# CatchMan1/AI-education-generative-recommendation

Hardware: AMD Instinct MI355X
Metric: RQ-VAE items encoded/s + SASRec seqs scored/s @1/8 GPU; HR@10/NDCG@10 parity (higher is better)
Workload: dtype f32; 1 GPU; rq_c2: RQ-VAE get_indices, 3x256 codebooks, in 768 -> [256,128] -> e 32, data-derived codebooks, BERT-statistics item embeddings; global_batch=100000, parallelism=item-sharded x1, no collective

## Files before the change

### ai-education-generative-recommendation_amd/csrc/rq_fused.hip

```cpp
#include <type_traits>

#include "gr_common.h"

#ifndef GR_EDIAG
#define GR_EDIAG 0
#endif

namespace gr {

constexpr int FT = 32;
constexpr int FP = 2;
constexpr int FXC = 64;
constexpr int FXP = FXC + 4;
constexpr int FWV = 8;

template <int H1, int H2>
struct FusedCfg {
  static constexpr int E = 32;
  static constexpr int NTH = 64 * FWV;
  static constexpr int P1 = H1 + 4, P2 = H2 + 4, P3 = H2 + 4;
  static constexpr int PI = FP * FT;
  static constexpr int XV = PI * 16 / NTH;
  static constexpr int LDS = 2 * PI * FXP + PI * P1 + PI * P2 + E * P3;
  static_assert(H1 == 32 * FWV && H2 == 128, "8-wave form: H1 = 256, H2 = 128");
};

__device__ __forceinline__ f32x4 ldg4(const float* p) {
  return *reinterpret_cast<const __attribute__((address_space(1))) f32x4*>(reinterpret_cast<uintptr_t>(p));
}

__device__ __forceinline__ void put_packed(float* row, int k0, const f32x4& v) {
  const int g = k0 & ~31, q = k0 & 31, j = q >> 3, e2 = (q >> 1) & 2;
  *reinterpret_cast<f32x2*>(row + g + 4 * j + e2) = f32x2{v[0], v[2]};
  *reinterpret_cast<f32x2*>(row + g + 16 + 4 * j + e2) = f32x2{v[1], v[3]};
}

__device__ __forceinline__ int xrow(int f) { return ((f >> 7) << 3) + ((f >> 5) & 3) + 4 * ((f >> 4) & 1); }

template <int H1, int H2>
struct FusedCtx {
  using C = FusedCfg<H1, H2>;
  const float* x;
  int64_t n;
  int D0, NC, csplit, t_end;
  const float *W2, *b1, *b2, *W3, *b3;
  float* z_out;
  float *xs, *h1s, *h2s, *w3s;
  int tid, w, r, h;
  const float* w1row;
  f32x4 awc[4];
  f32x4 awc2[4];
  f32x4 w2f[4];
  f32x4 xr[C::XV];
  bool xok[C::XV];
  f32x4 bxa[4];
  int buf;
  __device__ __forceinline__ void gload_x(int tb, int c, bool ks) {
#pragma unroll
    for (int i = 0; i < C::XV; ++i) {
      const int f = tid + C::NTH * i, it = xrow(f), k4 = (f & 15) * 4;
      const int64_t item = (int64_t)tb * FT + (ks ? it % FT : it);
      xok[i] = item < n && (ks || (tb + it / FT) < t_end);
      xr[i] = *reinterpret_cast<const f32x4*>(x + (item < n ? item : n - 1) * D0 +
                                              (int64_t)c * FXC + k4 + (ks && it >= FT ? csplit * FXC : 0));
    }
  }
  __device__ __forceinline__ void read_bxa(int g) {
    const float* xb = xs + buf * C::PI * FXP + r * FXP + 16 * h + g * 32;
#pragma unroll
    for (int j = 0; j < 4; ++j) bxa[j] = *reinterpret_cast<const f32x4*>(xb + 4 * j);
  }
  __device__ __forceinline__ void swrite_x(int b) {
#pragma unroll
    for (int i = 0; i < C::XV; ++i) {
      const int f = tid + C::NTH * i;
      put_packed(xs + b * C::PI * FXP + xrow(f) * FXP, (f & 15) * 4,
                 xok[i] ? xr[i] : f32x4{0.f, 0.f, 0.f, 0.f});
    }
  }
};

__device__ __forceinline__ int h1_swz(int row) { return ((row >> 2) ^ (row >> 3)) & 1; }

__device__ __forceinline__ void store_h1(float* row, int x, int g4, int h, const f32x4& o) {
  float* p = row + 16 * (g4 >> 1) + 2 * (g4 & 1) + h;
#pragma unroll
  for (int i = 0; i < 4; ++i) p[4 * (i ^ x)] = o[i];
}

template <int NR, int H1, int H2>
__device__ __forceinline__ void rq_l23(FusedCtx<H1, H2>& cx, int tb) {
#pragma clang fp contract(off)
  using C = FusedCfg<H1, H2>;
  constexpr int E = C::E, P1 = C::P1, P2 = C::P2;
  const int w = cx.w, lane = cx.tid & 63, j = lane & 15, g = lane >> 4;
  f32x4 bb3;
  {
    constexpr int NT = 2 * NR, UB = 4, NI = H1 / (16 * UB);
    f32x4 acc2[NT];
#pragma unroll
    for (int it = 0; it < NT; ++it) acc2[it] = f32x4{0.f, 0.f, 0.f, 0.f};
    const float* hb = cx.h1s + j * P1 + 4 * (g ^ h1_swz(j));
    const float* w2row = cx.W2 + (int64_t)(w * 16 + j) * H1 + 4 * g;
    f32x4 aw2[UB];
#pragma unroll
    for (int u = 0; u < UB; ++u) aw2[u] = cx.w2f[u];
    const f32x4 bb = ldg4(cx.b2 + w * 16 + 4 * g);
    bb3 = ldg4(cx.b3 + 16 * (w & 1) + 4 * g);
    asm volatile("" ::: "memory");
#pragma unroll 1
    for (int bi = 0; bi < (GR_EDIAG == 1 ? 0 : NI); ++bi) {
      const int bn = (bi + 1 < NI) ? bi + 1 : bi;
      f32x4 awn[UB];
#pragma unroll
      for (int u = 0; u < UB; ++u) awn[u] = ldg4(w2row + 16 * (bn * UB + u));
      f32x4 bx[UB][NT];
#pragma unroll
      for (int u = 0; u < UB; ++u)
#pragma unroll
        for (int it = 0; it < NT; ++it)
          bx[u][it] = *reinterpret_cast<const f32x4*>(hb + it * 16 * P1 + 16 * (bi * UB + u));
#pragma unroll
      for (int u = 0; u < UB; ++u)
#pragma unroll
        for (int t = 0; t < 4; ++t)
#pragma unroll
          for (int it = 0; it < NT; ++it) acc2[it] = mfma16(aw2[u][t], bx[u][it][t], acc2[it]);
      __builtin_amdgcn_sched_group_barrier(0x100, NT, 0);
#pragma unroll
      for (int i = 0; i < UB; ++i) {
        __builtin_amdgcn_sched_group_barrier(0x008, 1, 0);
        __builtin_amdgcn_sched_group_barrier(0x020, 1, 0);
      }
#pragma unroll
      for (int i = 0; i < (UB - 1) * NT; ++i) {
        __builtin_amdgcn_sched_group_barrier(0x008, 1, 0);
        __builtin_amdgcn_sched_group_barrier(0x100, 1, 0);
      }
      __builtin_amdgcn_sched_group_barrier(0x008, 4 * UB * NT - UB - (UB - 1) * NT, 0);
#pragma unroll
      for (int u = 0; u < UB; ++u) aw2[u] = awn[u];
    }
#pragma unroll
    for (int it = 0; it < NT; ++it) {
      float* row = cx.h2s + (it * 16 + j) * P2 + w * 16 + g;
#pragma unroll
      for (int i = 0; i < 4; ++i) {
        const float u = bb[i] + acc2[it][i];
        row[4 * i] = u < 0.f ? 0.f : u;
      }
    }
  }
  __syncthreads();

  if (GR_EDIAG != 2 && w < 4 * NR) {
    const int it = w >> 2, ih = (w >> 1) & 1, oh = w & 1;
    f32x4 acc3 = {0.f, 0.f, 0.f, 0.f};
    const float* hb = cx.h2s + (it * FT + 16 * ih + j) * P2 + 4 * g;
    const float* w3row = cx.w3s + (16 * oh + j) * C::P3 + 4 * g;
#pragma unroll
    for (int b = 0; b < H2 / 16; ++b) {
      const f32x4 aw = *reinterpret_cast<const f32x4*>(w3row + 16 * b);
      const f32x4 bx = *reinterpret_cast<const f32x4*>(hb + 16 * b);
#pragma unroll
      for (int t = 0; t < 4; ++t) acc3 = mfma16(aw[t], bx[t], acc3);
    }
    const int64_t item = (int64_t)(tb + it) * FT + 16 * ih + j;
    if (item < cx.n) {
      f32x4 o;
#pragma unroll
      for (int i = 0; i < 4; ++i) o[i] = bb3[i] + acc3[i];
      *reinterpret_cast<f32x4*>(cx.z_out + item * E + 16 * oh + 4 * g) = o;
    }
  }
}

template <int NP, int H1, int H2, bool KS = false>
__device__ __forceinline__ void rq_fused_pass(FusedCtx<H1, H2>& cx, int tb, int next_tb, bool next_ks) {
#pragma clang fp contract(off)
  using C = FusedCfg<H1, H2>;
  constexpr int P1 = C::P1, PI = C::PI;
  static_assert(!KS || NP == 2, "k-split pass: two chains");
  constexpr int NR = KS ? 1 : NP;
  const int w = cx.w, r = cx.r, h = cx.h;
  const int NC = KS ? cx.NC / 2 : cx.NC;
  const int kbo = cx.csplit * FXC;
  asm volatile("" : "+s"(cx.W2), "+s"(cx.W3), "+s"(cx.b1), "+s"(cx.b2), "+s"(cx.b3));

  f32x16 acc1[NP];
#pragma unroll
  for (int it = 0; it < NP; ++it)
#pragma unroll
    for (int v = 0; v < 16; ++v) acc1[it][v] = 0.f;
  constexpr int M1 = 16 * NP;
  const float* xsrc[C::XV];
  const float* xnxt[C::XV];
  bool xok_cur[C::XV], xok_nxt[C::XV];
#pragma unroll
  for (int i = 0; i < C::XV; ++i) {
    const int f = cx.tid + C::NTH * i, it = xrow(f), k4 = (f & 15) * 4;
    const int64_t a = (int64_t)tb * FT + (KS ? it % FT : it);
    const int64_t b = next_tb < 0 ? cx.n : (int64_t)next_tb * FT + (next_ks ? it % FT : it);
    xsrc[i] = cx.x + (a < cx.n ? a : cx.n - 1) * cx.D0 + k4 + (KS && it >= FT ? kbo : 0);
    xnxt[i] = cx.x + (b < cx.n ? b : cx.n - 1) * cx.D0 + k4 + (next_ks && it >= FT ? kbo : 0);
    xok_cur[i] = a < cx.n;
    xok_nxt[i] = b < cx.n && (next_ks || (next_tb + it / FT) < cx.t_end);
    if (b >= cx.n) xnxt[i] = cx.x + (cx.n - 1) * cx.D0 + k4;
  }
  auto group = [&](auto gsel, int c) {
    constexpr int g = decltype(gsel)::value;
    const int gi = 2 * c + g;
    const int gn = (gi + 1 == 2 * NC) ? 0 : gi + 1;
    f32x4 awn[4], awn2[4];
#pragma unroll
    for (int j = 0; j < 4; ++j) awn[j] = *reinterpret_cast<const f32x4*>(cx.w1row + gn * 32 + 4 * j);
    if constexpr (KS) {
#pragma unroll
      for (int j = 0; j < 4; ++j) awn2[j] = *reinterpret_cast<const f32x4*>(cx.w1row + kbo + gn * 32 + 4 * j);
    }
    const float* xb = cx.xs + cx.buf * PI * FXP + r * FXP + 16 * h + g * 32;
    f32x4 bx[NP][4];
#pragma unroll
    for (int j = 0; j < 4; ++j) bx[0][j] = cx.bxa[j];
#pragma unroll
    for (int it = 1; it < NP; ++it)
#pragma unroll
      for (int j = 0; j < 4; ++j) bx[it][j] = *reinterpret_cast<const f32x4*>(xb + it * FT * FXP + 4 * j);
    if constexpr (g == 0) {
      cx.read_bxa(1);
      asm volatile("" ::: "memory");
      const bool same = c + 1 < NC;
#pragma unroll
      for (int i = 0; i < C::XV; ++i)
        cx.xr[i] = *reinterpret_cast<const f32x4*>(same ? xsrc[i] + (c + 1) * FXC : xnxt[i]);
    }
#pragma unroll
    for (int it = 0; it < NP; ++it)
#pragma unroll
      for (int j = 0; j < 4; ++j)
#pragma unroll
        for (int s = 0; s < 4; ++s)
          acc1[it] = mfma32(KS && it == 1 ? cx.awc2[j][s] : cx.awc[j][s], bx[it][j][s], acc1[it]);
    if constexpr (g == 1) {
      const bool same = c + 1 < NC;
#pragma unroll
      for (int i = 0; i < C::XV; ++i) {
        const int f = cx.tid + C::NTH * i;
        const bool ok = same ? xok_cur[i] : xok_nxt[i];
        put_packed(cx.xs + (cx.buf ^ 1) * PI * FXP + xrow(f) * FXP, (f & 15) * 4,
                   ok ? cx.xr[i] : f32x4{0.f, 0.f, 0.f, 0.f});
      }
    }
    constexpr int NX = (g == 0) ? C::XV : 0, NDW = (g == 1) ? 2 * C::XV : 0;
    constexpr int NW = KS ? 8 : 4, NA = (g == 0) ? 4 : 0;
    static_assert(NW + 4 * (NP - 1) + NA + NX + 2 * NDW <= M1, "schedule");
    {
#pragma unroll
      for (int i = 0; i < NW; ++i) {
        __builtin_amdgcn_sched_group_barrier(0x008, 1, 0);
        __builtin_amdgcn_sched_group_barrier(0x020, 1, 0);
      }
#pragma unroll
      for (int i = 0; i < 4 * (NP - 1) + NA; ++i) {
        __builtin_amdgcn_sched_group_barrier(0x008, 1, 0);
        __builtin_amdgcn_sched_group_barrier(0x100, 1, 0);
      }
#pragma unroll
      for (int i = 0; i < NX; ++i) {
        __builtin_amdgcn_sched_group_barrier(0x008, 1, 0);
        __builtin_amdgcn_sched_group_barrier(0x020, 1, 0);
      }
      __builtin_amdgcn_sched_group_barrier(0x008, M1 - NW - 4 * (NP - 1) - NA - NX - 2 * NDW, 0);
#pragma unroll
      for (int i = 0; i < NDW; ++i) {
        __builtin_amdgcn_sched_group_barrier(0x008, 1, 0);
        __builtin_amdgcn_sched_group_barrier(0x200, 1, 0);
      }
    }
#pragma unroll
    for (int j = 0; j < 4; ++j) cx.awc[j] = awn[j];
    if constexpr (KS) {
#pragma unroll
      for (int j = 0; j < 4; ++j) cx.awc2[j] = awn2[j];
    }
  };
  const int f0 = w * 32;
  auto chunk = [&](int c) {
    group(std::integral_constant<int, 0>{}, c);
    group(std::integral_constant<int, 1>{}, c);
    __syncthreads();
    cx.buf ^= 1;
    cx.read_bxa(0);
    __builtin_amdgcn_sched_group_barrier(0x100, 4, 0);
    __builtin_amdgcn_sched_group_barrier(0x008, 2 * C::XV, 0);
  };
  int c = 0;
  f32x16 part[NP];
  f32x4 b1f[4];
#pragma unroll
  for (int g4 = 0; g4 < 4; ++g4) b1f[g4] = ldg4(cx.b1 + f0 + 8 * g4 + 4 * h);
  asm volatile("" ::: "memory");
  if constexpr (KS) {
#pragma unroll
    for (int j = 0; j < 4; ++j) cx.awc2[j] = *reinterpret_cast<const f32x4*>(cx.w1row + kbo + 4 * j);
#pragma unroll 1
    for (; c < NC; ++c) chunk(c);
#pragma unroll
    for (int g4 = 0; g4 < 4; ++g4) {
      const f32x4 bb = b1f[g4];
#pragma unroll
      for (int i = 0; i < 4; ++i) part[0][4 * g4 + i] = bb[i] + acc1[0][4 * g4 + i];
    }
#pragma unroll
    for (int v = 0; v < 16; ++v) acc1[0][v] = acc1[1][v];
  } else {
#pragma unroll 1
    for (; c < cx.csplit; ++c) chunk(c);
#pragma unroll
    for (int g4 = 0; g4 < 4; ++g4) {
      const f32x4 bb = b1f[g4];
#pragma unroll
      for (int it = 0; it < NP; ++it)
#pragma unroll
        for (int i = 0; i < 4; ++i) part[it][4 * g4 + i] = bb[i] + acc1[it][4 * g4 + i];
    }
#pragma unroll
    for (int it = 0; it < NP; ++it)
#pragma unroll
      for (int v = 0; v < 16; ++v) acc1[it][v] = 0.f;
#pragma unroll 1
    for (; c < NC; ++c) chunk(c);
  }
#pragma unroll
  for (int g4 = 0; g4 < 4; ++g4)
#pragma unroll
    for (int it = 0; it < NR; ++it) {
      f32x4 o;
#pragma unroll
      for (int i = 0; i < 4; ++i) {
        const float u = part[it][4 * g4 + i] + acc1[it][4 * g4 + i];
        o[i] = u < 0.f ? 0.f : u;
      }
      store_h1(cx.h1s + (it * FT + r) * P1 + f0, h1_swz(r), g4, h, o);
    }
  __syncthreads();

  rq_l23<NR, H1, H2>(cx, tb);
}

template <int H1, int H2, int PF = 128>
__device__ __forceinline__ void rq_piece_pass(FusedCtx<H1, H2>& cx, int tb, int fh, float* __restrict__ h1g,
                                              const float* __restrict__ W1) {
#pragma clang fp contract(off)
  using C = FusedCfg<H1, H2>;
  constexpr int PI = C::PI;
  constexpr int NG = PF / 32;
  const int w = cx.w, r = cx.r, h = cx.h, fg = w % NG, blk = (w / NG) & 1;
  const bool act = w < 2 * NG;
  const int NC = cx.NC / 2, kbo = cx.csplit * FXC;
  const int f0 = PF * fh + 32 * fg;
  const float* w1row = W1 + (int64_t)(f0 + r) * cx.D0 + 16 * h + blk * kbo;
  f32x4 awc[4];
#pragma unroll
  for (int j = 0; j < 4; ++j) awc[j] = act ? *reinterpret_cast<const f32x4*>(w1row + 4 * j) : f32x4{0.f, 0.f, 0.f, 0.f};
  const float* xsrc[C::XV];
  bool xok[C::XV];
#pragma unroll
  for (int i = 0; i < C::XV; ++i) {
    const int f = cx.tid + C::NTH * i, it = xrow(f), k4 = (f & 15) * 4;
    const int64_t a = (int64_t)tb * FT + it % FT;
    xsrc[i] = cx.x + (a < cx.n ? a : cx.n - 1) * cx.D0 + k4 + (it >= FT ? kbo : 0);
    xok[i] = a < cx.n;
  }
  f32x16 acc;
#pragma unroll
  for (int v = 0; v < 16; ++v) acc[v] = 0.f;
#pragma unroll 1
  for (int c = 0; c < NC; ++c) {
    const bool more = c + 1 < NC;
#pragma unroll
    for (int g = 0; g < 2; ++g) {
      const int gi = 2 * c + g;
      const int gn = gi + 1 < 2 * NC ? gi + 1 : gi;
      f32x4 awn[4];
#pragma unroll
      for (int j = 0; j < 4; ++j)
        awn[j] = act ? *reinterpret_cast<const f32x4*>(w1row + gn * 32 + 4 * j) : f32x4{0.f, 0.f, 0.f, 0.f};
      const float* xb = cx.xs + cx.buf * PI * FXP + (blk * FT + r) * FXP + 16 * h + g * 32;
      f32x4 bx[4];
#pragma unroll
      for (int j = 0; j < 4; ++j) bx[j] = *reinterpret_cast<const f32x4*>(xb + 4 * j);
      if (g == 0 && more) {
#pragma unroll
        for (int i = 0; i < C::XV; ++i) cx.xr[i] = *reinterpret_cast<const f32x4*>(xsrc[i] + (c + 1) * FXC);
      }
      if (act) {
#pragma unroll
        for (int j = 0; j < 4; ++j)
#pragma unroll
          for (int s = 0; s < 4; ++s) acc = mfma32(awc[j][s], bx[j][s], acc);
      }
      if (g == 1 && more) {
#pragma unroll
        for (int i = 0; i < C::XV; ++i) {
          const int f = cx.tid + C::NTH * i;
          put_packed(cx.xs + (cx.buf ^ 1) * PI * FXP + xrow(f) * FXP, (f & 15) * 4,
                     xok[i] ? cx.xr[i] : f32x4{0.f, 0.f, 0.f, 0.f});
        }
      }
#pragma unroll
      for (int j = 0; j < 4; ++j) awc[j] = awn[j];
    }
    __syncthreads();
    cx.buf ^= 1;
  }
  float* hand = cx.h1s + (fg * 64 + (cx.tid & 63)) * 16;
  if (act && blk == 1) {
#pragma unroll
    for (int v4 = 0; v4 < 4; ++v4)
      *reinterpret_cast<f32x4*>(hand + 4 * v4) = f32x4{acc[4 * v4], acc[4 * v4 + 1], acc[4 * v4 + 2], acc[4 * v4 + 3]};
  }
  __syncthreads();
  if (act && blk == 0) {
    const int64_t item = (int64_t)tb * FT + r;
#pragma unroll
    for (int g4 = 0; g4 < 4; ++g4) {
      const f32x4 bb = ldg4(cx.b1 + f0 + 8 * g4 + 4 * h);
      const f32x4 a1 = *reinterpret_cast<const f32x4*>(hand + 4 * g4);
      f32x4 o;
#pragma unroll
      for (int i = 0; i < 4; ++i) {
        const float part = bb[i] + acc[4 * g4 + i];
        const float u = part + a1[i];
        o[i] = u < 0.f ? 0.f : u;
      }
      if (item < cx.n) *reinterpret_cast<f32x4*>(h1g + (int64_t)r * H1 + f0 + 8 * g4 + 4 * h) = o;
    }
  }
  __syncthreads();
}

template <int H1, int H2>
__global__ __launch_bounds__(64 * FWV, 1) void rq_encoder_kernel(
    const float* __restrict__ x, int64_t n, int D0, int csplit, const float* __restrict__ W1,
    const float* __restrict__ b1, const float* __restrict__ W2, const float* __restrict__ b2,
    const float* __restrict__ W3, const float* __restrict__ b3, float* __restrict__ z_out,
    int tiles, float* __restrict__ h1g, int pq) {
  using C = FusedCfg<H1, H2>;
  extern __shared__ __attribute__((aligned(16))) float sm[];
  const int G = gridDim.x, q = tiles / G, b = blockIdx.x;
  const int npieces = (h1g && GR_EDIAG != 3) ? pq * (tiles - q * G) : 0;
  const int t_begin = h1g ? b * q : (int)((int64_t)b * tiles / G);
  const int t_end = h1g ? t_begin + q : (int)((int64_t)(b + 1) * tiles / G);
  const int piece0 = b < npieces ? b : -1;
  const bool pieces_only = t_begin >= t_end;
  if (pieces_only && piece0 < 0) return;
  FusedCtx<H1, H2> cx;
  cx.x = x; cx.n = n; cx.D0 = D0; cx.NC = D0 / FXC; cx.csplit = csplit; cx.t_end = t_end;
  cx.W2 = W2; cx.b1 = b1; cx.b2 = b2; cx.W3 = W3; cx.b3 = b3; cx.z_out = z_out;
  cx.xs = sm;
  cx.h1s = sm + 2 * C::PI * FXP;
  cx.h2s = cx.h1s + C::PI * C::P1;
  cx.w3s = cx.h2s + C::PI * C::P2;
  for (int f = threadIdx.x; f < C::E * H2 / 4; f += C::NTH) {
    const int row = f / (H2 / 4), qq = f % (H2 / 4);
    *reinterpret_cast<f32x4*>(cx.w3s + row * C::P3 + 4 * qq) = *reinterpret_cast<const f32x4*>(W3 + row * H2 + 4 * qq);
  }
  const int tid = threadIdx.x, lane = tid & 63;
  cx.tid = tid; cx.w = tid >> 6; cx.r = lane & 31; cx.h = lane >> 5;
  cx.w1row = W1 + (int64_t)(cx.w * 32 + cx.r) * D0 + 16 * cx.h;
#pragma unroll
  for (int j = 0; j < 4; ++j) cx.awc[j] = *reinterpret_cast<const f32x4*>(cx.w1row + 4 * j);
#pragma unroll
  for (int u = 0; u < 4; ++u)
    cx.w2f[u] = *reinterpret_cast<const f32x4*>(W2 + (int64_t)(cx.w * 16 + (lane & 15)) * H1 + 4 * (lane >> 4) + 16 * u);
  cx.buf = 0;
  const bool kso = 2 * csplit == cx.NC;
  const bool ks = kso && ((t_end - t_begin) & 1);
  const int ptile = piece0 >= 0 ? q * G + piece0 / pq : -1;
  cx.gload_x(pieces_only ? ptile : t_begin, 0, pieces_only || (ks && t_end - t_begin == 1));
  cx.swrite_x(0);
  __syncthreads();
  cx.read_bxa(0);
  int tb = t_begin;
  for (; tb + FP <= t_end; tb += FP) {
    const bool last = tb + FP >= t_end;
    rq_fused_pass<FP, H1, H2>(cx, tb, last ? ptile : tb + FP, last ? ptile >= 0 : ks && tb + FP + 1 == t_end);
  }
  if (tb < t_end) {
    if (ks) rq_fused_pass<2, H1, H2, true>(cx, tb, ptile, ptile >= 0);
    else rq_fused_pass<1, H1, H2>(cx, tb, ptile, ptile >= 0);
  }
  for (int pc = piece0; pc >= 0 && pc < npieces; pc += G) {
    const int t = q * G + pc / pq;
    if (pc != piece0) {
      cx.gload_x(t, 0, true);
      cx.swrite_x(cx.buf);
      __syncthreads();
    }
    float* dst = h1g + (int64_t)(pc / pq) * FT * H1;
    if (pq == 4) rq_piece_pass<H1, H2, 64>(cx, t, pc & 3, dst, W1);
    else rq_piece_pass<H1, H2, 128>(cx, t, pc & 1, dst, W1);
  }
}

template <int H1, int H2>
__global__ __launch_bounds__(64 * FWV) void rq_leftover_kernel(const float* __restrict__ h1g, int64_t n, int t0,
                                                          const float* __restrict__ W2, const float* __restrict__ b2,
                                                          const float* __restrict__ W3, const float* __restrict__ b3,
                                                          float* __restrict__ z_out) {
  using C = FusedCfg<H1, H2>;
  __shared__ __attribute__((aligned(16))) float h1s[FT * C::P1];
  __shared__ __attribute__((aligned(16))) float h2s[FT * C::P2];
  __shared__ __attribute__((aligned(16))) float w3s[C::E * C::P3];
  const int tid = threadIdx.x, lane = tid & 63;
  FusedCtx<H1, H2> cx;
#pragma unroll
  for (int u = 0; u < 4; ++u)
    cx.w2f[u] = *reinterpret_cast<const f32x4*>(W2 + (int64_t)((tid >> 6) * 16 + (lane & 15)) * H1 + 4 * (lane >> 4) + 16 * u);
  const float* src = h1g + (int64_t)blockIdx.x * FT * H1;
  for (int f = tid; f < FT * H1 / 4; f += C::NTH) {
    const int row = f / (H1 / 4), k0 = (f % (H1 / 4)) * 4;
    const f32x4 v = *reinterpret_cast<const f32x4*>(src + row * H1 + k0);
    float* p = h1s + row * C::P1 + (k0 & ~15) + ((k0 >> 2) & 3);
#pragma unroll
    for (int g = 0; g < 4; ++g) p[4 * (g ^ h1_swz(row))] = v[g];
  }
  for (int f = tid; f < C::E * H2 / 4; f += C::NTH) {
    const int row = f / (H2 / 4), qq = f % (H2 / 4);
    *reinterpret_cast<f32x4*>(w3s + row * C::P3 + 4 * qq) = *reinterpret_cast<const f32x4*>(W3 + row * H2 + 4 * qq);
  }
  __syncthreads();
  cx.n = n; cx.W2 = W2; cx.b2 = b2; cx.W3 = W3; cx.b3 = b3; cx.z_out = z_out;
  cx.h1s = h1s; cx.h2s = h2s; cx.w3s = w3s;
  cx.tid = tid; cx.w = tid >> 6; cx.r = lane & 31; cx.h = lane >> 5;
  rq_l23<1, H1, H2>(cx, t0 + blockIdx.x);
}

constexpr int PACK_IMAGES = 5;
struct PackArgs {
  const float* w[PACK_IMAGES];
  int64_t end[PACK_IMAGES];
  int K[PACK_IMAGES];
};
__global__ __launch_bounds__(256) void rq_pack_kernel(PackArgs a, float* __restrict__ out) {
  int64_t i = (int64_t)blockIdx.x * 256 + threadIdx.x;
  if (i >= a.end[PACK_IMAGES - 1]) return;
  int l = 0;
  while (i >= a.end[l]) ++l;
  const int64_t o = i - (l ? a.end[l - 1] : 0);
  const int K = a.K[l];
  const int64_t row = o / K;
  const int p = (int)(o % K);
  if (l >= 2) {
    const int b = p & ~15, g = (p >> 2) & 3, t = p & 3;
    out[i] = a.w[l][row * K + b + 4 * t + g];
    return;
  }
  const int g = p & ~31, q = p & 31, h = q >> 4, j = (q >> 2) & 3, s = q & 3;
  out[i] = a.w[l][row * K + g + 8 * j + 2 * s + h];
}

}

size_t gr_rq_fused_pack_floats(int32_t n_linear, const int32_t* dims) {
  if (n_linear != 3 || dims[3] != 32 || dims[1] != 256 || dims[2] != 128) return 0;
  return 2 * ((size_t)dims[0] * 256 + 256 * 128) + 128 * 32;
}

int gr_rq_encoder_pack_launch(int32_t n_linear, const int32_t* dims, const float* const* weights, float* pack,
                              hipStream_t st) {
  using namespace gr;
  if (gr_rq_fused_pack_floats(n_linear, dims) == 0) return GR_ERR_UNSUPPORTED;
  PackArgs pa{};
  int64_t tot = 0;
  for (int i = 0; i < PACK_IMAGES; ++i) {
    const int l = i < 3 ? i : i - 3;
    pa.w[i] = weights[l];
    pa.K[i] = dims[l];
    tot += (int64_t)dims[l + 1] * dims[l];
    pa.end[i] = tot;
  }
  hipLaunchKernelGGL(rq_pack_kernel, dim3((unsigned)((tot + 255) / 256)), dim3(256), 0, st, pa, pack);
  return check_launch("rq encoder pack");
}

int gr_rq_encoder_fused_launch(const float* x, int64_t n, int32_t n_linear, const int32_t* dims,
                               const float* const* weights, const float* const* biases,
                               float* z_out, float* pack, hipStream_t st, bool pack_is_ready, float* scratch) {
  using namespace gr;
  if (n_linear != 3 || dims[3] != 32 || dims[0] % FXC != 0 || !biases) return GR_ERR_UNSUPPORTED;
  if (!(dims[1] == 256 && dims[2] == 128)) return GR_ERR_UNSUPPORTED;
  const MklPlan p1 = mkl_plan(n, dims[0], 256);
  if (p1.kind != MKL_CHAIN || mkl_plan(n, 256, 128).kind != MKL_CHAIN || mkl_plan(n, 128, 32).kind != MKL_CHAIN)
    return GR_ERR_UNSUPPORTED;
  const int kb = p1.kb;
  if (2 * kb < dims[0] || (kb < dims[0] && kb % FXC != 0)) return GR_ERR_UNSUPPORTED;
  for (int i = 0; i < 3; ++i)
    if (!weights[i] || !biases[i] || !aligned16(biases[i])) return GR_ERR_UNSUPPORTED;
  if (!aligned16(x) || !aligned16(z_out) || !pack || !aligned16(pack)) return GR_ERR_UNSUPPORTED;
  if (n == 0) return GR_OK;
  const int64_t tiles = (n + FT - 1) / FT;
  if (tiles > 0x7fffffffLL) return fail(GR_ERR_UNSUPPORTED, "rq encoder: n too large");
  float* wp[3] = {pack, pack + (size_t)dims[0] * 256, pack + (size_t)dims[0] * 256 + 256 * 128};
  if (!pack_is_ready) {
    const int rc = gr_rq_encoder_pack_launch(n_linear, dims, weights, pack, st);
    if (rc) return rc;
  }
  static int cus = 0;
  if (!cus) {
    int dev = 0;
    if (hipGetDevice(&dev) != hipSuccess) dev = 0;
    if (hipDeviceGetAttribute(&cus, hipDeviceAttributeMultiprocessorCount, dev) != hipSuccess || cus < 1)
      cus = 256;
  }
  const int csplit = kb < dims[0] ? kb / FXC : dims[0] / FXC;
  const bool can_split = scratch && 2 * csplit * FXC == dims[0];
  const bool small = can_split && 4 * tiles <= cus;
  const int64_t grid = small ? 4 * tiles : tiles < cus ? tiles : cus;
  using Cfg = FusedCfg<256, 128>;
  static bool lds_ok = hipFuncSetAttribute(reinterpret_cast<const void*>(rq_encoder_kernel<256, 128>),
                                           hipFuncAttributeMaxDynamicSharedMemorySize,
                                           (int)(Cfg::LDS * sizeof(float))) == hipSuccess;
  if (!lds_ok) return fail(GR_ERR_HIP, "rq fused encoder: cannot raise the LDS limit");
  const int64_t left = small ? tiles : tiles % grid;
  float* h1g = (can_split && left) ? scratch : nullptr;
  const int pq = 4 * left <= grid ? 4 : 2;
  const float* w2t = wp[2] + 128 * 32 + (size_t)dims[0] * 256;
  hipLaunchKernelGGL((rq_encoder_kernel<256, 128>), dim3((unsigned)grid), dim3(64 * FWV), Cfg::LDS * sizeof(float), st, x, n,
                     dims[0], csplit, wp[0], biases[0], w2t, biases[1], wp[2], biases[2], z_out, (int)tiles, h1g, pq);
  int rc = check_launch("rq fused encoder");
  if (rc || !h1g || GR_EDIAG == 3) return rc;
  hipLaunchKernelGGL((rq_leftover_kernel<256, 128>), dim3((unsigned)left), dim3(64 * FWV), 0, st, h1g, n,
                     (int)(tiles - left), w2t, biases[1], wp[2], biases[2], z_out);
  return check_launch("rq fused encoder (leftover tiles)");
}
```

Measured before the change: 244.4 million items/s.

## Use buffer resource loads with hardware bounds clamping for x and W1 staging

Replaces per-thread 64-bit pointer arithmetic, clamping and validity flags for the x tile and W1 loads with AMD buffer resources whose size limits make out-of-range loads return zero. Precomputes LDS read and write pointers and swaps double buffers by flipping a pointer offset instead of recomputing addresses each time. The aim is to cut scalar and vector address ALU work and register pressure in the hot layer-1 loop. It adds a size guard on the input dimension and depends on buffer out-of-bounds semantics to produce zero padding correctly.

```diff
diff --git a/ai-education-generative-recommendation_amd/csrc/rq_fused.hip b/ai-education-generative-recommendation_amd/csrc/rq_fused.hip
--- a/ai-education-generative-recommendation_amd/csrc/rq_fused.hip
+++ b/ai-education-generative-recommendation_amd/csrc/rq_fused.hip
@@ -23,19 +23,37 @@
   static constexpr int XV = PI * 16 / NTH;
   static constexpr int LDS = 2 * PI * FXP + PI * P1 + PI * P2 + E * P3;
   static_assert(H1 == 32 * FWV && H2 == 128, "8-wave form: H1 = 256, H2 = 128");
+  static_assert(XV == FP, "x staging: a thread's float4 i is a row of item tile i (XSrc)");
 };
 
 __device__ __forceinline__ f32x4 ldg4(const float* p) {
   return *reinterpret_cast<const __attribute__((address_space(1))) f32x4*>(reinterpret_cast<uintptr_t>(p));
 }
 
-__device__ __forceinline__ void put_packed(float* row, int k0, const f32x4& v) {
+__device__ __forceinline__ int xrow(int f) { return ((f >> 7) << 3) + ((f >> 5) & 3) + 4 * ((f >> 4) & 1); }
+
+__device__ __forceinline__ int packed_pos(int k0) {
   const int g = k0 & ~31, q = k0 & 31, j = q >> 3, e2 = (q >> 1) & 2;
-  *reinterpret_cast<f32x2*>(row + g + 4 * j + e2) = f32x2{v[0], v[2]};
-  *reinterpret_cast<f32x2*>(row + g + 16 + 4 * j + e2) = f32x2{v[1], v[3]};
-}
-
-__device__ __forceinline__ int xrow(int f) { return ((f >> 7) << 3) + ((f >> 5) & 3) + 4 * ((f >> 4) & 1); }
+  return g + 4 * j + e2;
+}
+__device__ __forceinline__ void put_packed(float* p, const f32x4& v) {
+  p[0] = v[0];
+  p[16] = v[1];
+  p[1] = v[2];
+  p[17] = v[3];
+}
+
+using rsrc_t = __amdgpu_buffer_rsrc_t;
+__device__ __forceinline__ rsrc_t make_rsrc(const float* p, int bytes) {
+  return __builtin_amdgcn_make_buffer_rsrc(const_cast<float*>(p), 0, bytes, 0x00020000);
+}
+__device__ __forceinline__ f32x4 buf_ld4(rsrc_t rs, int voff, int soff) {
+  return __builtin_bit_cast(f32x4, __builtin_amdgcn_raw_buffer_load_b128(rs, voff, soff, 0));
+}
+
+struct XSrc {
+  rsrc_t half[2];
+};
 
 template <int H1, int H2>
 struct FusedCtx {
@@ -47,36 +65,48 @@
   float* z_out;
   float *xs, *h1s, *h2s, *w3s;
   int tid, w, r, h;
-  const float* w1row;
+  rsrc_t w1rs;
+  int w1vo;
   f32x4 awc[4];
   f32x4 awc2[4];
   f32x4 w2f[4];
   f32x4 xr[C::XV];
-  bool xok[C::XV];
   f32x4 bxa[4];
-  int buf;
-  __device__ __forceinline__ void gload_x(int tb, int c, bool ks) {
-#pragma unroll
-    for (int i = 0; i < C::XV; ++i) {
-      const int f = tid + C::NTH * i, it = xrow(f), k4 = (f & 15) * 4;
-      const int64_t item = (int64_t)tb * FT + (ks ? it % FT : it);
-      xok[i] = item < n && (ks || (tb + it / FT) < t_end);
-      xr[i] = *reinterpret_cast<const f32x4*>(x + (item < n ? item : n - 1) * D0 +
-                                              (int64_t)c * FXC + k4 + (ks && it >= FT ? csplit * FXC : 0));
-    }
+  int xvo;
+  const float* xrd;
+  float* xwr;
+  int xflip;
+  __device__ __forceinline__ void flip() {
+    xrd += xflip;
+    xwr -= xflip;
+    xflip = -xflip;
+  }
+  __device__ __forceinline__ XSrc xsrc_of(int tb, bool ks) const {
+    const int64_t row0 = (int64_t)(tb < 0 ? 0 : tb) * FT;
+    const int tl = ks ? 1 : (t_end - tb < FP ? t_end - tb : FP);
+    int64_t left = n - row0;
+    if (left > tl * FT) left = tl * FT;
+    const int rows = (tb < 0 || left < 0) ? 0 : (int)left;
+    const float* p = x + row0 * D0;
+    const int lo = rows < FT ? rows : FT;
+    XSrc s;
+    s.half[0] = make_rsrc(p, lo * D0 * 4);
+    s.half[1] = ks ? make_rsrc(p + csplit * FXC, lo * D0 * 4) : make_rsrc(p + (int64_t)FT * D0, (rows - lo) * D0 * 4);
+    return s;
+  }
+  __device__ __forceinline__ void gload_x(const XSrc& s, int soff) {
+#pragma unroll
+    for (int i = 0; i < C::XV; ++i) xr[i] = buf_ld4(s.half[i], xvo, soff);
   }
   __device__ __forceinline__ void read_bxa(int g) {
-    const float* xb = xs + buf * C::PI * FXP + r * FXP + 16 * h + g * 32;
+    const float* xb = xrd + g * 32;
 #pragma unroll
     for (int j = 0; j < 4; ++j) bxa[j] = *reinterpret_cast<const f32x4*>(xb + 4 * j);
   }
-  __device__ __forceinline__ void swrite_x(int b) {
-#pragma unroll
-    for (int i = 0; i < C::XV; ++i) {
-      const int f = tid + C::NTH * i;
-      put_packed(xs + b * C::PI * FXP + xrow(f) * FXP, (f & 15) * 4,
-                 xok[i] ? xr[i] : f32x4{0.f, 0.f, 0.f, 0.f});
-    }
+  __device__ __forceinline__ void swrite_x(bool cur = false) {
+    float* p = cur ? xwr - xflip : xwr;
+#pragma unroll
+    for (int i = 0; i < C::XV; ++i) put_packed(p + i * FT * FXP, xr[i]);
   }
 };
 
@@ -179,7 +209,7 @@
 __device__ __forceinline__ void rq_fused_pass(FusedCtx<H1, H2>& cx, int tb, int next_tb, bool next_ks) {
 #pragma clang fp contract(off)
   using C = FusedCfg<H1, H2>;
-  constexpr int P1 = C::P1, PI = C::PI;
+  constexpr int P1 = C::P1;
   static_assert(!KS || NP == 2, "k-split pass: two chains");
   constexpr int NR = KS ? 1 : NP;
   const int w = cx.w, r = cx.r, h = cx.h;
@@ -193,32 +223,19 @@
 #pragma unroll
     for (int v = 0; v < 16; ++v) acc1[it][v] = 0.f;
   constexpr int M1 = 16 * NP;
-  const float* xsrc[C::XV];
-  const float* xnxt[C::XV];
-  bool xok_cur[C::XV], xok_nxt[C::XV];
-#pragma unroll
-  for (int i = 0; i < C::XV; ++i) {
-    const int f = cx.tid + C::NTH * i, it = xrow(f), k4 = (f & 15) * 4;
-    const int64_t a = (int64_t)tb * FT + (KS ? it % FT : it);
-    const int64_t b = next_tb < 0 ? cx.n : (int64_t)next_tb * FT + (next_ks ? it % FT : it);
-    xsrc[i] = cx.x + (a < cx.n ? a : cx.n - 1) * cx.D0 + k4 + (KS && it >= FT ? kbo : 0);
-    xnxt[i] = cx.x + (b < cx.n ? b : cx.n - 1) * cx.D0 + k4 + (next_ks && it >= FT ? kbo : 0);
-    xok_cur[i] = a < cx.n;
-    xok_nxt[i] = b < cx.n && (next_ks || (next_tb + it / FT) < cx.t_end);
-    if (b >= cx.n) xnxt[i] = cx.x + (cx.n - 1) * cx.D0 + k4;
-  }
+  const XSrc xcur = cx.xsrc_of(tb, KS), xnxt = cx.xsrc_of(next_tb, next_ks);
   auto group = [&](auto gsel, int c) {
     constexpr int g = decltype(gsel)::value;
     const int gi = 2 * c + g;
     const int gn = (gi + 1 == 2 * NC) ? 0 : gi + 1;
     f32x4 awn[4], awn2[4];
 #pragma unroll
-    for (int j = 0; j < 4; ++j) awn[j] = *reinterpret_cast<const f32x4*>(cx.w1row + gn * 32 + 4 * j);
+    for (int j = 0; j < 4; ++j) awn[j] = buf_ld4(cx.w1rs, cx.w1vo, gn * 128 + 16 * j);
     if constexpr (KS) {
 #pragma unroll
-      for (int j = 0; j < 4; ++j) awn2[j] = *reinterpret_cast<const f32x4*>(cx.w1row + kbo + gn * 32 + 4 * j);
-    }
-    const float* xb = cx.xs + cx.buf * PI * FXP + r * FXP + 16 * h + g * 32;
+      for (int j = 0; j < 4; ++j) awn2[j] = buf_ld4(cx.w1rs, cx.w1vo, (kbo + gn * 32) * 4 + 16 * j);
+    }
+    const float* xb = cx.xrd + g * 32;
     f32x4 bx[NP][4];
 #pragma unroll
     for (int j = 0; j < 4; ++j) bx[0][j] = cx.bxa[j];
@@ -230,9 +247,9 @@
       cx.read_bxa(1);
       asm volatile("" ::: "memory");
       const bool same = c + 1 < NC;
-#pragma unroll
-      for (int i = 0; i < C::XV; ++i)
-        cx.xr[i] = *reinterpret_cast<const f32x4*>(same ? xsrc[i] + (c + 1) * FXC : xnxt[i]);
+      const int so = same ? (c + 1) * FXC * 4 : 0;
+#pragma unroll
+      for (int i = 0; i < C::XV; ++i) cx.xr[i] = buf_ld4(same ? xcur.half[i] : xnxt.half[i], cx.xvo, so);
     }
 #pragma unroll
     for (int it = 0; it < NP; ++it)
@@ -241,16 +258,7 @@
 #pragma unroll
         for (int s = 0; s < 4; ++s)
           acc1[it] = mfma32(KS && it == 1 ? cx.awc2[j][s] : cx.awc[j][s], bx[it][j][s], acc1[it]);
-    if constexpr (g == 1) {
-      const bool same = c + 1 < NC;
-#pragma unroll
-      for (int i = 0; i < C::XV; ++i) {
-        const int f = cx.tid + C::NTH * i;
-        const bool ok = same ? xok_cur[i] : xok_nxt[i];
-        put_packed(cx.xs + (cx.buf ^ 1) * PI * FXP + xrow(f) * FXP, (f & 15) * 4,
-                   ok ? cx.xr[i] : f32x4{0.f, 0.f, 0.f, 0.f});
-      }
-    }
+    if constexpr (g == 1) cx.swrite_x();
     constexpr int NX = (g == 0) ? C::XV : 0, NDW = (g == 1) ? 2 * C::XV : 0;
     constexpr int NW = KS ? 8 : 4, NA = (g == 0) ? 4 : 0;
     static_assert(NW + 4 * (NP - 1) + NA + NX + 2 * NDW <= M1, "schedule");
@@ -289,7 +297,7 @@
     group(std::integral_constant<int, 0>{}, c);
     group(std::integral_constant<int, 1>{}, c);
     __syncthreads();
-    cx.buf ^= 1;
+    cx.flip();
     cx.read_bxa(0);
     __builtin_amdgcn_sched_group_barrier(0x100, 4, 0);
     __builtin_amdgcn_sched_group_barrier(0x008, 2 * C::XV, 0);
@@ -302,7 +310,7 @@
   asm volatile("" ::: "memory");
   if constexpr (KS) {
 #pragma unroll
-    for (int j = 0; j < 4; ++j) cx.awc2[j] = *reinterpret_cast<const f32x4*>(cx.w1row + kbo + 4 * j);
+    for (int j = 0; j < 4; ++j) cx.awc2[j] = buf_ld4(cx.w1rs, cx.w1vo, kbo * 4 + 16 * j);
 #pragma unroll 1
     for (; c < NC; ++c) chunk(c);
 #pragma unroll
@@ -352,26 +360,17 @@
 __device__ __forceinline__ void rq_piece_pass(FusedCtx<H1, H2>& cx, int tb, int fh, float* __restrict__ h1g,
                                               const float* __restrict__ W1) {
 #pragma clang fp contract(off)
-  using C = FusedCfg<H1, H2>;
-  constexpr int PI = C::PI;
   constexpr int NG = PF / 32;
   const int w = cx.w, r = cx.r, h = cx.h, fg = w % NG, blk = (w / NG) & 1;
   const bool act = w < 2 * NG;
   const int NC = cx.NC / 2, kbo = cx.csplit * FXC;
   const int f0 = PF * fh + 32 * fg;
-  const float* w1row = W1 + (int64_t)(f0 + r) * cx.D0 + 16 * h + blk * kbo;
+  const int w1vo = act ? ((f0 + r) * cx.D0 + 16 * h + blk * kbo) * 4 : 0x7ffffff0;
   f32x4 awc[4];
 #pragma unroll
-  for (int j = 0; j < 4; ++j) awc[j] = act ? *reinterpret_cast<const f32x4*>(w1row + 4 * j) : f32x4{0.f, 0.f, 0.f, 0.f};
-  const float* xsrc[C::XV];
-  bool xok[C::XV];
-#pragma unroll
-  for (int i = 0; i < C::XV; ++i) {
-    const int f = cx.tid + C::NTH * i, it = xrow(f), k4 = (f & 15) * 4;
-    const int64_t a = (int64_t)tb * FT + it % FT;
-    xsrc[i] = cx.x + (a < cx.n ? a : cx.n - 1) * cx.D0 + k4 + (it >= FT ? kbo : 0);
-    xok[i] = a < cx.n;
-  }
+  for (int j = 0; j < 4; ++j) awc[j] = buf_ld4(cx.w1rs, w1vo, 16 * j);
+  const XSrc xcur = cx.xsrc_of(tb, true);
+  const int xbo = blk * FT * FXP;
   f32x16 acc;
 #pragma unroll
   for (int v = 0; v < 16; ++v) acc[v] = 0.f;
@@ -384,35 +383,24 @@
       const int gn = gi + 1 < 2 * NC ? gi + 1 : gi;
       f32x4 awn[4];
 #pragma unroll
-      for (int j = 0; j < 4; ++j)
-        awn[j] = act ? *reinterpret_cast<const f32x4*>(w1row + gn * 32 + 4 * j) : f32x4{0.f, 0.f, 0.f, 0.f};
-      const float* xb = cx.xs + cx.buf * PI * FXP + (blk * FT + r) * FXP + 16 * h + g * 32;
+      for (int j = 0; j < 4; ++j) awn[j] = buf_ld4(cx.w1rs, w1vo, gn * 128 + 16 * j);
+      const float* xb = cx.xrd + xbo + g * 32;
       f32x4 bx[4];
 #pragma unroll
       for (int j = 0; j < 4; ++j) bx[j] = *reinterpret_cast<const f32x4*>(xb + 4 * j);
-      if (g == 0 && more) {
-#pragma unroll
-        for (int i = 0; i < C::XV; ++i) cx.xr[i] = *reinterpret_cast<const f32x4*>(xsrc[i] + (c + 1) * FXC);
-      }
+      if (g == 0 && more) cx.gload_x(xcur, (c + 1) * FXC * 4);
       if (act) {
 #pragma unroll
         for (int j = 0; j < 4; ++j)
 #pragma unroll
           for (int s = 0; s < 4; ++s) acc = mfma32(awc[j][s], bx[j][s], acc);
       }
-      if (g == 1 && more) {
-#pragma unroll
-        for (int i = 0; i < C::XV; ++i) {
-          const int f = cx.tid + C::NTH * i;
-          put_packed(cx.xs + (cx.buf ^ 1) * PI * FXP + xrow(f) * FXP, (f & 15) * 4,
-                     xok[i] ? cx.xr[i] : f32x4{0.f, 0.f, 0.f, 0.f});
-        }
-      }
+      if (g == 1 && more) cx.swrite_x();
 #pragma unroll
       for (int j = 0; j < 4; ++j) awc[j] = awn[j];
     }
     __syncthreads();
-    cx.buf ^= 1;
+    cx.flip();
   }
   float* hand = cx.h1s + (fg * 64 + (cx.tid & 63)) * 16;
   if (act && blk == 1) {
@@ -468,18 +456,22 @@
   }
   const int tid = threadIdx.x, lane = tid & 63;
   cx.tid = tid; cx.w = tid >> 6; cx.r = lane & 31; cx.h = lane >> 5;
-  cx.w1row = W1 + (int64_t)(cx.w * 32 + cx.r) * D0 + 16 * cx.h;
-#pragma unroll
-  for (int j = 0; j < 4; ++j) cx.awc[j] = *reinterpret_cast<const f32x4*>(cx.w1row + 4 * j);
+  cx.w1rs = make_rsrc(W1, H1 * D0 * 4);
+  cx.w1vo = ((cx.w * 32 + cx.r) * D0 + 16 * cx.h) * 4;
+#pragma unroll
+  for (int j = 0; j < 4; ++j) cx.awc[j] = buf_ld4(cx.w1rs, cx.w1vo, 16 * j);
+  cx.xvo = (xrow(tid) * D0 + 4 * (tid & 15)) * 4;
+  cx.xrd = cx.xs + cx.r * FXP + 16 * cx.h;
+  cx.xwr = cx.xs + C::PI * FXP + xrow(tid) * FXP + packed_pos(4 * (tid & 15));
+  cx.xflip = C::PI * FXP;
 #pragma unroll
   for (int u = 0; u < 4; ++u)
     cx.w2f[u] = *reinterpret_cast<const f32x4*>(W2 + (int64_t)(cx.w * 16 + (lane & 15)) * H1 + 4 * (lane >> 4) + 16 * u);
-  cx.buf = 0;
   const bool kso = 2 * csplit == cx.NC;
   const bool ks = kso && ((t_end - t_begin) & 1);
   const int ptile = piece0 >= 0 ? q * G + piece0 / pq : -1;
-  cx.gload_x(pieces_only ? ptile : t_begin, 0, pieces_only || (ks && t_end - t_begin == 1));
-  cx.swrite_x(0);
+  cx.gload_x(cx.xsrc_of(pieces_only ? ptile : t_begin, pieces_only || (ks && t_end - t_begin == 1)), 0);
+  cx.swrite_x(true);
   __syncthreads();
   cx.read_bxa(0);
   int tb = t_begin;
@@ -494,8 +486,8 @@
   for (int pc = piece0; pc >= 0 && pc < npieces; pc += G) {
     const int t = q * G + pc / pq;
     if (pc != piece0) {
-      cx.gload_x(t, 0, true);
-      cx.swrite_x(cx.buf);
+      cx.gload_x(cx.xsrc_of(t, true), 0);
+      cx.swrite_x(true);
       __syncthreads();
     }
     float* dst = h1g + (int64_t)(pc / pq) * FT * H1;
@@ -591,6 +583,7 @@
   using namespace gr;
   if (n_linear != 3 || dims[3] != 32 || dims[0] % FXC != 0 || !biases) return GR_ERR_UNSUPPORTED;
   if (!(dims[1] == 256 && dims[2] == 128)) return GR_ERR_UNSUPPORTED;
+  if (dims[0] > (1 << 20)) return GR_ERR_UNSUPPORTED;
   const MklPlan p1 = mkl_plan(n, dims[0], 256);
   if (p1.kind != MKL_CHAIN || mkl_plan(n, 256, 128).kind != MKL_CHAIN || mkl_plan(n, 128, 32).kind != MKL_CHAIN)
     return GR_ERR_UNSUPPORTED;
```

Result: faster. 261.7 million items/s (median of 6 runs) (+7.1%).
